# mantasu/face-crop-plus

Measured on AMD Instinct MI355X. Metric: faces/sec end-to-end (detect+align+crop), higher is better.
Workload: dtype f16x3; 1 GPU; RetinaFace detect + 5-pt align/crop, batch=32/GPU synthetic 1024x1024 RGB, strategy=largest, det_threshold=0.6, output 256x256, detector on 2 HIP streams x 16 images; global_batch=32, image_size=1024, parallelism=dp1

## Files before the change

### face-crop-plus_amd/_native.py

```python
from __future__ import annotations

import ctypes as C
import os

_HERE = os.path.dirname(os.path.abspath(__file__))
LIB_PATH = os.path.join(_HERE, "csrc", "libfcp_hip.so")
ABI_VERSION = 15

c_f32p = C.c_void_p
_lib = None


class ConvDesc(C.Structure):
    _fields_ = [
        ("in_", C.c_void_p), ("w", C.c_void_p), ("bias", C.c_void_p), ("out", C.c_void_p),
        ("res1", C.c_void_p), ("res2", C.c_void_p), ("wscale", C.c_void_p), ("in2", C.c_void_p),
        ("n", C.c_int32), ("in_h", C.c_int32), ("in_w", C.c_int32),
        ("cin", C.c_int32), ("in_ld", C.c_int32), ("in_up2", C.c_int32),
        ("cout", C.c_int32), ("kh", C.c_int32), ("kw", C.c_int32),
        ("stride", C.c_int32), ("pad", C.c_int32),
        ("out_h", C.c_int32), ("out_w", C.c_int32), ("out_ld", C.c_int32),
        ("tile_n", C.c_int32), ("cin4", C.c_int32),
        ("act_slope", C.c_float), ("alpha", C.c_float), ("alpha2", C.c_float),
        ("res1_pre", C.c_int32), ("res1_ld", C.c_int32), ("res1_h", C.c_int32),
        ("res1_w", C.c_int32), ("res2_ld", C.c_int32), ("precision", C.c_int32),
        ("in_fmt", C.c_int32), ("out_fmt", C.c_int32), ("res1_fmt", C.c_int32), ("res2_fmt", C.c_int32),
        ("tile_m", C.c_int32), ("cin2", C.c_int32), ("in2_ld", C.c_int32), ("in2_h", C.c_int32),
        ("in2_w", C.c_int32), ("in2_stride", C.c_int32), ("flags", C.c_int32), ("cu_budget", C.c_int32),
        ("band_top", C.c_int32), ("band_bottom", C.c_int32),
    ]


CONV_FLAT_ADDR = 1
CONV_BALANCE_TAIL = 2
CHAIN_OUT_EVEN_ONLY = 1


class ChainDesc(C.Structure):
    _fields_ = [(k, C.c_void_p) for k in ("t1", "w2", "ws2", "b2", "w3", "ws3", "b3", "res", "out", "w1n", "ws1n",
                                          "b1n", "t1n", "t1b")] + \
               [(k, C.c_int32) for k in ("n", "h", "w", "c", "cn", "t1_ld", "res_ld", "out_ld", "t1n_ld", "nout", "tile_m", "flags",
                                         "cb", "t1b_ld", "t1b_h", "t1b_w", "t1b_stride")]


_P, _I, _F, _L = C.c_void_p, C.c_int, C.c_float, C.c_int64
SIGNATURES = {
    "fcp_conv2d_nhwc_f32": [C.POINTER(ConvDesc), _P],
    "fcp_bottleneck_chain_f16x3": [C.POINTER(ChainDesc), _P],
    "fcp_u8_to_nhwc4_f32": [_P, _P, _L, C.POINTER(C.c_float), _F, _P],
# ... 83 lines not shown
```

### face-crop-plus_amd/csrc/fcp_conv.hip

```cpp
#include "fcp_conv_common.h"

#include <cstdlib>

using namespace fcp_conv;

namespace {

constexpr int LDK = 32;


typedef unsigned int u32x4 __attribute__((ext_vector_type(4)));

__device__ __forceinline__ f32x4 buf_load16(__amdgpu_buffer_rsrc_t rsrc, unsigned voff) {
  return __builtin_bit_cast(f32x4, __builtin_amdgcn_raw_buffer_load_b128(rsrc, (int)voff, 0, 0));
}

template <int BN, bool CIN4, bool BUF>
__global__ void __launch_bounds__(256, (BN == 128 ? 2 : (BN == 64 ? 3 : 4))) conv_igemm_f32(const ConvK p) {
  constexpr int WAVES_N = (BN == 32) ? 1 : 2;
  constexpr int WAVES_M = 4 / WAVES_N;
  constexpr int WTM = BM / WAVES_M;
  constexpr int WTN = BN / WAVES_N;
  constexpr int TM = WTM / 32, TN = WTN / 32;
  constexpr int A_LD = BM / 32;
// ... 211 lines not shown
                (!d->res1 || (d->res1_h == d->out_h && d->res1_w == d->out_w)) || halo_wide,
                "conv: the halo-tile kernel needs a 3x3 / stride 1 / pad 1 conv with cin >= 64, cout <= 64 (cout %% 8 == 0) on the "
                "fp16x3 path with a split32 input, no second source, no resized residual");
  if (halo_wide)
    FCP_REQUIRE(d->precision == 1 && d->in_fmt == 1 && !d->cin4 && d->kh == 3 && d->kw == 3 && d->stride == 1 &&
                d->pad == 1 && d->cout % 8 == 0 && d->cin >= 64 && d->cin % 64 == 0 && !d->in2 &&
                ((d->tile_n == 64 && d->cout <= 64 && (!d->res1 || (d->res1_h == d->out_h && d->res1_w == d->out_w))) ||
                 (d->tile_n == 128 && d->cout <= 128 && !d->res1 && !d->res2)),
                "conv: the wide halo-tile kernel (tile_m 1, tile_n 64 / 128) needs a 3x3 / stride 1 / pad 1 conv with cin %% 64 == 0, "
                "cout <= tile_n (cout %% 8 == 0; no residuals above 64 filters) on the fp16x3 path with a split32 input");
  FCP_REQUIRE(d->tile_n == 32 || d->tile_n == 64 || d->tile_n == 128 || (big && (d->tile_n == 256 || d->tile_n == 192)),
              "conv: tile_n must be 32/64/128 (or 192 / 256 with tile_m 256)");
  if (big)
    FCP_REQUIRE(d->precision == 1 && d->in_fmt == 1 && !d->cin4 && !d->in_up2 && d->cout % 8 == 0 && d->tile_n >= 128,
                "conv: 256-row tiles need the fp16x3 path on a split32 input (no cin4 / in_up2), cout %% 8 == 0, tile_n 128/256");
  FCP_REQUIRE(d->kh >= 1 && d->kw >= 1 && d->stride >= 1 && d->pad >= 0, "conv: bad filter geometry");
  FCP_REQUIRE(d->kh * d->kw <= 32 || d->cin4, "conv: at most 32 filter taps (kh*kw) outside cin4 mode");
  FCP_REQUIRE(d->in_ld % 4 == 0 && ((uintptr_t)d->in & 15) == 0, "conv: input must be 16-byte aligned, in_ld %% 4 == 0");
  FCP_REQUIRE(((uintptr_t)d->w & 15) == 0, "conv: filter must be 16-byte aligned");
  if (d->cin4) {
    FCP_REQUIRE(d->cin <= 4 && d->in_ld == 4 && d->kw <= 8, "conv: cin4 mode needs cin<=4, in_ld==4, kw<=8");
  } else {
    FCP_REQUIRE(d->cin % 32 == 0 && d->cin > 0, "conv: cin must be a multiple of 32 (got %d)", d->cin);
  }
  FCP_REQUIRE(d->band_top >= 0 && d->band_bottom >= 0 && d->band_top <= d->pad && d->band_bottom <= d->pad &&
              ((d->band_top | d->band_bottom) == 0 || (d->stride == 1 && !d->in2)),
              "conv: band_top / band_bottom must lie in 0..pad (stride-1 convs without a second source only)");
  const int eh = (d->in_h - d->band_top - d->band_bottom + 2 * d->pad - d->kh) / d->stride + 1;
  const int ew = (d->in_w + 2 * d->pad - d->kw) / d->stride + 1;
  FCP_REQUIRE(eh == d->out_h && ew == d->out_w, "conv: output size %dx%d does not match geometry %dx%d",
// ... 39 lines not shown
    FCP_REQUIRE(d->res1_h > 0 && d->res1_w > 0 && d->res1_ld > 0, "conv: res1 geometry missing");
    if (d->res1_h != d->out_h || d->res1_w != d->out_w) {
      k.res1_resize = 1;
      k.res1_sh = (float)d->res1_h / (float)d->out_h;
      k.res1_sw = (float)d->res1_w / (float)d->out_w;
    }
  }
  if (d->res2) FCP_REQUIRE(d->res2_ld > 0, "conv: res2_ld missing");
  k.vec_ok = (d->out_ld % 4 == 0) && (((uintptr_t)d->out & 15) == 0);
  if (d->res1) k.vec_ok = k.vec_ok && (d->res1_ld % 4 == 0) && (((uintptr_t)d->res1 & 15) == 0);
  if (d->res2) k.vec_ok = k.vec_ok && (d->res2_ld % 4 == 0) && (((uintptr_t)d->res2 & 15) == 0);
  static const int nt_env = getenv("FCP_NT_STORE") ? atoi(getenv("FCP_NT_STORE")) : 1;
  k.nt_store = nt_env;
  k.balance = (d->flags & FCP_CONV_BALANCE_TAIL) ? 1 : 0;
  k.cu_budget = d->cu_budget;
  k.mfull = 0; k.tail_rows = 0; k.round_size = 0;
  k.in2 = nullptr; k.in2_bytes = 0; k.csplit = d->cin; k.in2_ld = 0; k.ph2 = 0; k.pw2 = 0; k.stride2 = 1;
  if (d->in2) {
    FCP_REQUIRE(d->precision == 1 && d->in_fmt == 1 && !d->cin4 && !d->in_up2 && d->kh == 1 && d->kw == 1 && d->pad == 0,
                "conv: a second source needs a 1x1 / pad 0 conv on the fp16x3 path with split32 inputs");
    FCP_REQUIRE(d->cin2 > 0 && d->cin2 < d->cin && d->cin2 % 32 == 0 && d->in2_ld % 32 == 0 && d->in2_ld >= d->cin2 &&
                ((uintptr_t)d->in2 & 127) == 0, "conv: in2 must be a 32-channel-group aligned split32 view, 0 < cin2 < cin");
    FCP_REQUIRE(d->in2_stride >= 1 && d->in2_h > 0 && d->in2_w > 0 && (long)(d->out_h - 1) * d->in2_stride < d->in2_h &&
                (long)(d->out_w - 1) * d->in2_stride < d->in2_w, "conv: in2 geometry does not cover the output grid");
    const unsigned long in2_bytes = (unsigned long)d->n * d->in2_h * d->in2_w * d->in2_ld * 4ul;
    FCP_REQUIRE(in2_bytes < 0xFFFFFFF0ul, "conv: in2 must be below 4 GiB");
    k.in2 = d->in2; k.in2_bytes = (unsigned)in2_bytes; k.csplit = d->cin - d->cin2; k.in2_ld = d->in2_ld;
    k.ph2 = d->in2_h; k.pw2 = d->in2_w; k.stride2 = d->in2_stride;
  }
  k.grid_m = fcp_cdiv(M, BM);
  k.grid_n = fcp_cdiv(d->cout, d->tile_n);
// ... 8 lines not shown
    FCP_REQUIRE(d->wscale != nullptr, "conv: precision 1 needs wscale");
    k.in_bytes = (unsigned)in_bytes;
    k.w_bytes = (unsigned)w_bytes;
    if (halo) {
      k.grid_n = 1;
      const unsigned long out_bytes = (unsigned long)M * d->out_ld * 4ul;
      FCP_REQUIRE(out_bytes < 0xFFFFFFF0ul, "conv(halo): the output view must span less than 4 GiB");
      FCP_REQUIRE(d->wscale != nullptr && ((uintptr_t)d->wscale & 15) == 0 && ((uintptr_t)d->bias & 15) == 0,
                  "conv(halo): wscale / bias must be 16-byte aligned");
      k.in2_bytes = (unsigned)out_bytes;
      k.w_bytes = (unsigned)((unsigned long)fcp_cdiv(d->cout, 128) * 128ul * k.wrow * 4ul);
      return halo_wide ? launch_f16x3_halo_wide(k, s) : launch_f16x3_halo(k, s);
    }
    if (big) {
      k.w_bytes = (unsigned)((unsigned long)fcp_cdiv(d->cout, 128) * 128ul * k.wrow * 4ul);
      return launch_f16x3_big(k, d->tile_n, s);
    }
    if (k.in_fmt == 1 && !d->cin4) return launch_f16x3_dma(k, d->tile_n, s);
    return launch_f16x3(k, d->tile_n, d->cin4 != 0, s);
  }
  k.in_bytes = buf ? (unsigned)in_bytes : 0u;
  k.w_bytes = buf ? (unsigned)w_bytes : 0u;
#define FCP_DISPATCH(BN_)                                                             \
  do {                                                                                \
    if (d->cin4) return buf ? launch<BN_, true, true>(k, s) : launch<BN_, true, false>(k, s); \
    return buf ? launch<BN_, false, true>(k, s) : launch<BN_, false, false>(k, s);   \
  } while (0)
  switch (d->tile_n) {
    case 32: FCP_DISPATCH(32);
    case 64: FCP_DISPATCH(64);
// ... 5 lines not shown
```

### face-crop-plus_amd/csrc/fcp_conv_common.h

```cpp
#pragma once
#include <type_traits>
#include "fcp_common.h"
#include "fcp_hip.h"

typedef float f32x16 __attribute__((ext_vector_type(16)));
typedef float f32x4 __attribute__((ext_vector_type(4)));


constexpr int FCP_AUX_A = 0;
constexpr int FCP_AUX_B = 0;

namespace fcp_conv {

constexpr int BM = 128;
constexpr int BK = 32;

struct ConvK {
  const float* in;
  const float* w;
  const float* bias;
  float* out;
  const float* res1;
  const float* res2;
  int n, in_h, in_w, ph, pw, cin, in_ld, in_up2;
// ... 3 lines not shown
  float act_slope, alpha, alpha2;
  int res1_pre, res1_ld, res1_h, res1_w, res1_resize, res2_ld;
  float res1_sh, res1_sw;
  int grid_m, grid_n, vec_ok;
  unsigned in_bytes, w_bytes;
  const float* wscale;
  int in_fmt, out_fmt, res1_fmt, res2_fmt;
  const float* in2;
  unsigned in2_bytes;
  int csplit, in2_ld, ph2, pw2, stride2;
  int nt_store;
  int balance, cu_budget;
  int mfull, tail_rows, round_size;
  int big_tiles;
  int big_persist;
};


struct TapPiece {
  unsigned base, mask;
};

template <bool CIN4>
__device__ __forceinline__ TapPiece make_tap_piece(const ConvK& p, unsigned pbase, int hi0, int wi0, unsigned chan_off) {
  TapPiece t;
  t.base = ((pbase + (unsigned)(hi0 * p.pw + wi0)) * (unsigned)p.in_ld + chan_off) * 4u;
  t.mask = 0u;
  const int taps = CIN4 ? p.kh : p.kh * p.kw;
  for (int q = 0; q < taps; ++q) {
    const int kh_i = CIN4 ? q : q / p.kw;
// ... 202 lines not shown
        r.a[g] = *reinterpret_cast<const u32x4_t*>(p.res1 + m * p.res1_ld + co);
        r.b[g] = *reinterpret_cast<const u32x4_t*>(p.res1 + m * p.res1_ld + co + 4);
      }
    }
  }
}

template <int I, int N, typename F>
__device__ __forceinline__ void fcp_static_for(F&& f) {
  if constexpr (I < N) {
    f(std::integral_constant<int, I>{});
    fcp_static_for<I + 1, N>(f);
  }
}

template <int TM, int TN, int WTM, int WTN>
__device__ __forceinline__ void conv_epilogue_regs(const ConvK& p, f32x16 (&acc)[TM][TN], int m_start, int m_end, int tm_act, int co_tile,
                                                   int co_end, int wm, int wn, int lane, int hw) {
    const int lp = lane & 15, lg = lane >> 4;
  auto swap32 = [](float& x, float& y) {
    const auto r = __builtin_amdgcn_permlane32_swap(__float_as_uint(x), __float_as_uint(y), false, false);
    const unsigned r0 = r[0], r1 = r[1];
    x = __uint_as_float(r0); y = __uint_as_float(r1);
  };
  auto swap16 = [](float& x, float& y) {
    const auto r = __builtin_amdgcn_permlane16_swap(__float_as_uint(x), __float_as_uint(y), false, false);
    const unsigned r0 = r[0], r1 = r[1];
    x = __uint_as_float(r0); y = __uint_as_float(r1);
  };
  constexpr int GI = TM < 2 ? TM : 2;
  constexpr int NGI = (TM + GI - 1) / GI;
  constexpr int NG = TN * NGI;
  u32x4_t pend_a[GI][2], pend_b[GI][2];
  auto row_of = [&](int i, int set) { return m_start + wm * WTM + i * 32 + 16 * set + lp; };
  auto chan_of = [&](int jj) { return co_tile + wn * WTN + jj * 32 + 8 * lg; };
  auto flush = [&](auto gc) {
    constexpr int g = decltype(gc)::value, jj = g / NGI, i0 = (g % NGI) * GI;
    const int co = chan_of(jj);
    fcp_static_for<0, GI>([&](auto ic) {
      constexpr int i = i0 + decltype(ic)::value;
      if constexpr (i < TM) {
        fcp_static_for<0, 2>([&](auto sc) {
          constexpr int set = decltype(sc)::value;
          const int mi = row_of(i, set);
          if (i < tm_act && mi < m_end && co < co_end) {
            if (p.out_fmt == 1) {
              char* ob = reinterpret_cast<char*>(p.out) + (long)mi * p.out_ld * 4 + split_chan_off(co);
              *reinterpret_cast<u32x4_t*>(ob) = pend_a[i - i0][set];
              *reinterpret_cast<u32x4_t*>(ob + 64) = pend_b[i - i0][set];
            } else {
              float* dst = p.out + (long)mi * p.out_ld + co;
              *reinterpret_cast<u32x4_t*>(dst) = pend_a[i - i0][set];
              *reinterpret_cast<u32x4_t*>(dst + 4) = pend_b[i - i0][set];
            }
          }
        });
      }
    });
  };
  fcp_static_for<0, NG>([&](auto gc) {
    constexpr int g = decltype(gc)::value, j = g / NGI, i0 = (g % NGI) * GI;
    const int co = chan_of(j);
    const bool cok = co < co_end;
    const int cc = cok ? co : co_tile;
    u32x4_t r1a[GI][2], r1b[GI][2];
    if (p.res1 != nullptr) {
      fcp_static_for<0, GI>([&](auto ic) {
        constexpr int i = i0 + decltype(ic)::value;
        if constexpr (i < TM) {
          fcp_static_for<0, 2>([&](auto sc) {
            constexpr int set = decltype(sc)::value;
            const int mi = row_of(i, set);
            const long m = (i < tm_act && mi < m_end && cok) ? (long)mi : (long)m_start;
            long rpix = m;
            if (p.res1_resize) {
              const int ni = (int)(m / hw);
              const int rem = (int)(m - (long)ni * hw);
              const int ho = rem / p.out_w;
              const int wo = rem - ho * p.out_w;
              int sh = (int)floorf(ho * p.res1_sh);
              int sw = (int)floorf(wo * p.res1_sw);
              sh = sh < p.res1_h - 1 ? sh : p.res1_h - 1;
              sw = sw < p.res1_w - 1 ? sw : p.res1_w - 1;
              rpix = ((long)ni * p.res1_h + sh) * p.res1_w + sw;
            }
            if (p.res1_fmt == 1) {
              const char* pb = reinterpret_cast<const char*>(p.res1) + rpix * p.res1_ld * 4 + split_chan_off(cc);
              r1a[i - i0][set] = *reinterpret_cast<const u32x4_t*>(pb);
// ... 32 lines not shown
        });
        fcp_static_for<0, 2>([&](auto sc) {
          constexpr int set = decltype(sc)::value;
          float (&v)[8] = set == 0 ? va : vb;
          float r1[8], r2[8];
          if (p.res1 != nullptr) {
            if (p.res1_fmt == 1) {
              join8(r1a[i - i0][set], r1b[i - i0][set], r1);
            } else {
              const f32x4 fa = __builtin_bit_cast(f32x4, r1a[i - i0][set]), fb = __builtin_bit_cast(f32x4, r1b[i - i0][set]);
              r1[0] = fa[0]; r1[1] = fa[1]; r1[2] = fa[2]; r1[3] = fa[3]; r1[4] = fb[0]; r1[5] = fb[1]; r1[6] = fb[2]; r1[7] = fb[3];
            }
          }
          if (p.res2 != nullptr) {
            const int mi = row_of(i, set);
            load8(p.res2, (i < tm_act && mi < m_end && cok) ? (long)mi : (long)m_start, p.res2_ld, cc, p.res2_fmt, r2);
          }
#pragma unroll
          for (int e = 0; e < 8; ++e) {
            float x = v[e] * ws8[e] + bias8[e];
            if (p.res1 != nullptr && p.res1_pre) x += r1[e];
            x = x >= 0.f ? x : x * p.act_slope;
            x = x * p.alpha;
            if (p.res1 != nullptr && !p.res1_pre) x += r1[e];
            if (p.res2 != nullptr) x = x * p.alpha2 + r2[e];
            v[e] = x;
          }
          if (p.out_fmt == 1) {
            split8(f32x4{v[0], v[1], v[2], v[3]}, f32x4{v[4], v[5], v[6], v[7]}, pend_a[i - i0][set], pend_b[i - i0][set]);
          } else {
            pend_a[i - i0][set] = __builtin_bit_cast(u32x4_t, f32x4{v[0], v[1], v[2], v[3]});
// ... 113 lines not shown
```

### face-crop-plus_amd/csrc/fcp_conv_f16x3_big.hip

```cpp
#include "fcp_conv_common.h"

#include <type_traits>

using namespace fcp_conv;

namespace {

typedef _Float16 f16x8 __attribute__((ext_vector_type(8)));

constexpr int BMB = 256;
constexpr int NT = 512;
constexpr int ROWB = 128;
constexpr int STAGE = 1 << 16;

template <int IMM>
__device__ __forceinline__ f16x8 lds_read128(unsigned addr) {
  f16x8 v;
  asm volatile("ds_read_b128 %0, %1 offset:%2" : "=v"(v) : "v"(addr), "n"(IMM));
  return v;
}

template <int I, int N, typename F>
__device__ __forceinline__ void static_for(F&& f) {
  if constexpr (I < N) {
    f(std::integral_constant<int, I>{});
    static_for<I + 1, N>(f);
  }
}

template <int BN>
__global__ void __launch_bounds__(NT, 1) conv_igemm_f16x3_big(const ConvK p) {
  constexpr int WAVES_N = BN == 256 ? 4 : 2;
  constexpr int WAVES_M = 8 / WAVES_N;
  constexpr int WTM = BMB / WAVES_M, WTN = BN / WAVES_N;
  constexpr int TM = WTM / 32, TN = WTN / 32;
  constexpr int A_LD = BMB / 64, B_LD = BN / 64;

  extern __shared__ __attribute__((aligned(16))) float smem[];
  char* lds = reinterpret_cast<char*>(smem);

  const int nb = p.big_tiles;
  int vb = blockIdx.x;
  int tile_n = 0, m_start = 0, m_end = 0;
  auto decode = [&](int bid) {
    const int rbase = (bid / p.round_size) * p.round_size;
    const int nr = nb - rbase < p.round_size ? nb - rbase : p.round_size;
    const int bi = bid - rbase;
    const int q8 = nr >> 3, r8 = nr & 7, xcd = bi & 7;
    const int logical = rbase + (xcd < r8 ? xcd * (q8 + 1) : r8 * (q8 + 1) + (xcd - r8) * q8) + (bi >> 3);
    tile_n = logical % p.grid_n;
    const int tile_m = logical / p.grid_n;
// ... 2 lines not shown
    m_end = m_start + m_rows < p.M ? m_start + m_rows : p.M;
  };
  decode(vb);

  const int tid = threadIdx.x;
  const int lane = tid & 63;
  const int wave_u = __builtin_amdgcn_readfirstlane(tid >> 6);
  const int wm = wave_u / WAVES_N, wn = wave_u % WAVES_N;
  const int lrow = tid >> 3;
  const int csrc = (tid & 7) ^ (((lrow >> 1) & 7) ^ ((lrow & 1) << 2));

  const int hw = p.out_h * p.out_w;
  TapPiece tp[A_LD];
  unsigned base2[A_LD];
  unsigned woff[B_LD];
  auto setup_tile = [&]() {
#pragma unroll
  for (int i = 0; i < A_LD; ++i) {
    const int m = m_start + lrow + 64 * i;
    unsigned pbase = 0;
    int hi0 = -(1 << 28), wi0 = 0;
    base2[i] = 0xFFFFFFFFu;
    if (m < m_end) {
      const int ni = m / hw;
      const int rem = m - ni * hw;
      const int ho = rem / p.out_w;
      const int wo = rem - ho * p.out_w;
      pbase = (unsigned)(ni * p.ph * p.pw);
      hi0 = ho * p.stride - p.pad_h;
      wi0 = wo * p.stride - p.pad;
      if (p.in2 != nullptr)
        base2[i] = (((unsigned)(ni * p.ph2 + ho * p.stride2) * (unsigned)p.pw2 + (unsigned)(wo * p.stride2)) * (unsigned)p.in2_ld +
                    (unsigned)(csrc * 4)) * 4u;
    }
    tp[i] = make_tap_piece<false>(p, pbase, hi0, wi0, (unsigned)(csrc * 4));
  }
#pragma unroll
    for (int i = 0; i < B_LD; ++i) woff[i] = (unsigned)(((tile_n * BN + lrow + 64 * i) * p.wrow + csrc * 4) * 4);
  };
  setup_tile();
  __amdgpu_buffer_rsrc_t rs_in2 = __builtin_amdgcn_make_buffer_rsrc(const_cast<float*>(p.in2 ? p.in2 : p.in), 0, p.in2_bytes, 0x00020000);
  __amdgpu_buffer_rsrc_t rs_in = __builtin_amdgcn_make_buffer_rsrc(const_cast<float*>(p.in), 0, p.in_bytes, 0x00020000);
  __amdgpu_buffer_rsrc_t rs_w = __builtin_amdgcn_make_buffer_rsrc(const_cast<float*>(p.w), 0, p.w_bytes, 0x00020000);
  unsigned rowoff[A_LD];
  auto set_tap = [&](int tap, int kh_i, int kw_i) {
    const unsigned tapoff = (unsigned)((kh_i * p.pw + kw_i) * p.in_ld) * 4u;
#pragma unroll
    for (int i = 0; i < A_LD; ++i) rowoff[i] = ((tp[i].mask >> tap) & 1u) ? tp[i].base + tapoff : 0xFFFFFFFFu;
  };
  int tap = 0, kh_i = 0, kw_i = 0, c0 = 0;
  auto advance = [&]() {
// ... 16 lines not shown
      }
    } else {
#pragma unroll
      for (int i = 0; i < A_LD; ++i) {
        const unsigned ro = rowoff[i];
        __builtin_amdgcn_raw_ptr_buffer_load_lds(rs_in, (__attribute__((address_space(3))) void*)(a + 64 * i * ROWB), 16,
                                                 (int)(ro == 0xFFFFFFFFu ? 0xFFFFFFFFu : ro + (unsigned)(c0 * 4)), 0, 0, FCP_AUX_A);
      }
    }
#pragma unroll
    for (int i = 0; i < B_LD; ++i)
      __builtin_amdgcn_raw_ptr_buffer_load_lds(rs_w, (__attribute__((address_space(3))) void*)(b + 64 * i * ROWB), 16,
                                               (int)(woff[i] + (unsigned)(kt * BK * 4)), 0, 0, FCP_AUX_B);
  };

  f32x16 acc[TM][TN];

  const unsigned lds0 = (unsigned)(size_t)(__attribute__((address_space(3))) char*)lds;
  const int rsw = (((lane & 31) >> 1) & 7) ^ ((lane & 1) << 2);
  const int half = lane >> 5;
  const unsigned arow = lds0 + (unsigned)((wm * WTM + (lane & 31)) * ROWB);
  const unsigned brow = lds0 + (unsigned)((BMB + wn * WTN + (lane & 31)) * ROWB);
  unsigned aH[2], aL[2], bH[2], bL[2];
#pragma unroll
  for (int s = 0; s < 2; ++s) {
    const unsigned oh = (unsigned)(((2 * s + half) ^ rsw) << 4), ol = (unsigned)(((4 + 2 * s + half) ^ rsw) << 4);
    aH[s] = arow + oh; aL[s] = arow + ol;
    bH[s] = brow + oh; bL[s] = brow + ol;
  }

  auto prefetch_tile = [&]() {
    tap = 0; kh_i = 0; kw_i = 0; c0 = 0;
    set_tap(0, 0, 0);
    dma_slice(0, 0);
    if (p.ktiles > 1) {
      advance();
      dma_slice(1, 1);
    }
  };
  prefetch_tile();
  int tm_act = 0;
  auto main_loop = [&](auto tma_c) {
    constexpr int TMA = decltype(tma_c)::value;
    f16x8 fah[2][TMA > 0 ? TMA : 1], fal[2][TMA > 0 ? TMA : 1], fbh[2][TN], fbl[2][TN];
  auto read_frags = [&](auto set_c, unsigned stage_xor) {
    constexpr int set = decltype(set_c)::value;
    static_for<0, TMA>([&](auto ic) {
      constexpr int i = decltype(ic)::value;
      fah[set][i] = lds_read128<i * 32 * ROWB>(aH[set] ^ stage_xor);
      fal[set][i] = lds_read128<i * 32 * ROWB>(aL[set] ^ stage_xor);
    });
    static_for<0, TN>([&](auto jc) {
      constexpr int j = decltype(jc)::value;
      fbh[set][j] = lds_read128<j * 32 * ROWB>(bH[set] ^ stage_xor);
      fbl[set][j] = lds_read128<j * 32 * ROWB>(bL[set] ^ stage_xor);
    });
  };
  constexpr std::integral_constant<int, 0> SET0{};
  constexpr std::integral_constant<int, 1> SET1{};
  auto mfmas_reads = [&](auto cs_c, auto ls_c, unsigned stage_xor) {
    constexpr int cs = decltype(cs_c)::value, ls = decltype(ls_c)::value;
    constexpr int NM = 3 * TMA * TN, NR = 2 * TMA + 2 * TN;
    static_for<0, NM>([&](auto mc) {
      constexpr int m = decltype(mc)::value;
      constexpr int g = m / (TMA * TN), i = (m % (TMA * TN)) / TN, j = m % TN;
      if constexpr (g == 0) acc[i][j] = __builtin_amdgcn_mfma_f32_32x32x16_f16(fbh[cs][j], fal[cs][i], acc[i][j], 0, 0, 0);
      else if constexpr (g == 1) acc[i][j] = __builtin_amdgcn_mfma_f32_32x32x16_f16(fbl[cs][j], fah[cs][i], acc[i][j], 0, 0, 0);
      else acc[i][j] = __builtin_amdgcn_mfma_f32_32x32x16_f16(fbh[cs][j], fah[cs][i], acc[i][j], 0, 0, 0);
      __builtin_amdgcn_sched_barrier(0);
      static_for<0, NR>([&](auto rc) {
        constexpr int r = decltype(rc)::value;
        if constexpr (((r + 1) * NM) / NR - 1 == m
        ) {
          if constexpr (r < 2 * TMA) {
            constexpr int ii = r / 2;
            if constexpr (r % 2 == 0) fah[ls][ii] = lds_read128<ii * 32 * ROWB>(aH[ls] ^ stage_xor);
            else fal[ls][ii] = lds_read128<ii * 32 * ROWB>(aL[ls] ^ stage_xor);
          } else {
            constexpr int jj = (r - 2 * TMA) / 2;
            if constexpr (r % 2 == 0) fbh[ls][jj] = lds_read128<jj * 32 * ROWB>(bH[ls] ^ stage_xor);
            else fbl[ls][jj] = lds_read128<jj * 32 * ROWB>(bL[ls] ^ stage_xor);
          }
          __builtin_amdgcn_sched_barrier(0);
        }
      });
    });
  };

  read_frags(SET0, 0u);
  asm volatile("s_waitcnt lgkmcnt(0)" ::: "memory");
  __builtin_amdgcn_sched_barrier(0);

  unsigned sx = 0u;
  for (int kt = 0; kt < p.ktiles; ++kt) {
    mfmas_reads(SET0, SET1, sx);
    __builtin_amdgcn_sched_barrier(0);
    asm volatile("s_waitcnt lgkmcnt(0)" ::: "memory");
    asm volatile("s_waitcnt vmcnt(0)" ::: "memory");
    __builtin_amdgcn_s_barrier();
    __builtin_amdgcn_sched_barrier(0);
    const bool dma_first = wave_u >= 4;
    if (dma_first && kt + 2 < p.ktiles) {
      advance();
      dma_slice(kt + 2, kt & 1);
    }
    __builtin_amdgcn_sched_barrier(0);
    mfmas_reads(SET1, SET0, sx ^ (unsigned)STAGE);
    __builtin_amdgcn_sched_barrier(0);
    if (!dma_first && kt + 2 < p.ktiles) {
      advance();
      dma_slice(kt + 2, kt & 1);
    }
    __builtin_amdgcn_sched_barrier(0);
    asm volatile("s_waitcnt lgkmcnt(0)" ::: "memory");
    __builtin_amdgcn_sched_barrier(0);
    sx ^= (unsigned)STAGE;
  }
  };
  for (;;) {
  asm volatile("s_waitcnt vmcnt(0)" ::: "memory");
  __builtin_amdgcn_s_barrier();
  __builtin_amdgcn_sched_barrier(0);
  tm_act = (m_end - m_start - wm * WTM + 31) >> 5;
  tm_act = __builtin_amdgcn_readfirstlane(tm_act < 0 ? 0 : (tm_act > TM ? TM : tm_act));
#pragma unroll
  for (int i = 0; i < TM; ++i)
#pragma unroll
    for (int j = 0; j < TN; ++j)
#pragma unroll
      for (int e = 0; e < 16; ++e) acc[i][j][e] = 0.f;
  static_for<0, TM + 1>([&](auto tc) {
    if (tm_act == decltype(tc)::value) main_loop(tc);
  });
  asm volatile("s_waitcnt vmcnt(0)" ::: "memory");
  __builtin_amdgcn_s_barrier();

  const int e_tile_n = tile_n, e_m_start = m_start, e_m_end = m_end, e_tm_act = tm_act;
  const bool more = p.big_persist && vb + p.round_size < nb;
  if (more) {
    vb += p.round_size;
    decode(vb);
    setup_tile();
    prefetch_tile();
  }
  conv_epilogue_regs<TM, TN, WTM, WTN>(p, acc, e_m_start, e_m_end, e_tm_act, e_tile_n * BN,
                                       (e_tile_n + 1) * BN < p.cout ? (e_tile_n + 1) * BN : p.cout, wm, wn, lane, hw);
  if (!more) break;
  }
}

template <int BN>
int launch(ConvK k, hipStream_t s) {
  const size_t lds = 2 * (size_t)STAGE;
  FCP_LDS_OPT_IN((&conv_igemm_f16x3_big<BN>), lds);
  k.grid_n = fcp_cdiv(k.cout, BN);
  int cus = k.cu_budget > 0 ? k.cu_budget : fcp_cu_count();
  cus = cus < 8 ? 8 : (cus & ~7);
  k.round_size = cus;
  const int mt = fcp_cdiv(k.M, BMB);
  k.mfull = mt;
  k.tail_rows = BMB;
  k.grid_m = mt;
  if (k.balance) {
    const long tiles = (long)mt * k.grid_n;
    const long full_rounds = tiles / cus;
    const int mfull = (int)((full_rounds * cus) / k.grid_n);
    const long rem = (long)k.M - (long)mfull * BMB;
    if (rem > 0) {
      const long slots = cus / k.grid_n > 0 ? cus / k.grid_n : 1;
      long r = ((rem + slots - 1) / slots + 31) / 32 * 32;
      r = r < 32 ? 32 : r;
      if (r < BMB) {
        k.mfull = mfull;
        k.tail_rows = (int)r;
        k.grid_m = mfull + (int)((rem + r - 1) / r);
      }
    }
  }
  k.big_tiles = k.grid_m * k.grid_n;
  static const int persist_env = getenv("FCP_BIG_PERSIST") ? atoi(getenv("FCP_BIG_PERSIST")) : -1;
  k.big_persist = persist_env < 0 ? (k.cu_budget == 0) : (persist_env != 0);
  hipLaunchKernelGGL((conv_igemm_f16x3_big<BN>), dim3(k.big_persist && k.big_tiles > k.round_size ? k.round_size : k.big_tiles), dim3(NT), lds, s, k);
  FCP_LAUNCH_OK();
  return 0;
}

}

namespace fcp_conv {

int launch_f16x3_big(const ConvK& k, int tile_n, hipStream_t s) {
  return tile_n == 256 ? launch<256>(k, s) : tile_n == 192 ? launch<192>(k, s) : launch<128>(k, s);
}

}
```

### face-crop-plus_amd/engine.py

```python
from __future__ import annotations

import contextlib
import ctypes as C
import os
import threading
from dataclasses import dataclass

import numpy as np
import torch

from . import _native as N
from . import torch_ops as T

BN_EPS = 1e-5
COUT_PAD = 128


class Act:
    __slots__ = ("buf", "c0", "c", "fmt")

    def __init__(self, buf: torch.Tensor, c0: int = 0, c: int | None = None, fmt: int = 0):
        assert buf.dim() == 4 and buf.dtype == torch.float32 and buf.is_contiguous()
        self.buf, self.c0, self.fmt = buf, c0, fmt
        self.c = buf.shape[3] - c0 if c is None else c
# ... 564 lines not shown
    d.flags = flags
    d.cu_budget = cu_budget
    d.band_top, d.band_bottom = band
    if res1 is not None:
        d.res1_ld, d.res1_h, d.res1_w = res1.ld, res1.h, res1.w
    if res2 is not None:
        d.res2_ld = res2.ld
    return d


def conv(pc: PackedConv, x: Act, out: Act | None = None, *, act_slope: float = 1.0,
         alpha: float = 1.0, res1: Act | None = None, res1_pre: bool = True,
         res2: Act | None = None, alpha2: float = 1.0, in_up2: bool = False,
         tile_n: int | None = None, out_fmt: int = 0, tile_m: int | None = None,
         x2: Act | None = None, x2_stride: int = 1, flat: bool = False, balance_tail: bool = False,
         band: tuple[int, int] = (0, 0)) -> Act:
    assert x.c + (x2.c if x2 is not None else 0) == pc.cin, f"conv expects {pc.cin} input channels, got {x.c}"
    in_h, in_w = (x.h * 2, x.w * 2) if in_up2 else (x.h, x.w)
    oh = (in_h - band[0] - band[1] + 2 * pc.pad - pc.kh) // pc.stride + 1
    ow = (in_w + 2 * pc.pad - pc.kw) // pc.stride + 1
    if out is None:
        out = Act.empty(x.n, oh, ow, pc.cout, x.buf.device, out_fmt)
    assert (out.n, out.h, out.w, out.c) == (x.n, oh, ow, pc.cout), "conv: bad output view"
    if (x.fmt or out.fmt or (res1 is not None and res1.fmt) or (res2 is not None and res2.fmt)) and pc.precision != 1:
        raise ValueError("split32 tensors can only be used with filters packed for the fp16x3 path")
    assert x2 is None or (x2.fmt == 1 and x.fmt == 1 and x2.n == x.n), "two-source convs take split32 tensors"
    assert res1 is None or (res1.c == pc.cout and res1.n == x.n)
    assert res2 is None or (res2.n, res2.h, res2.w, res2.c) == (x.n, oh, ow, pc.cout)
    m = x.n * oh * ow
    tm, tn = tile_m or 128, tile_n or _pick_tile_n(pc.cout, m)
    flags = (N.CONV_FLAT_ADDR if flat else 0) | (N.CONV_BALANCE_TAIL if balance_tail else 0)
    cu = getattr(_budget, "cus", 0)
    desc = lambda o: _conv_desc(pc, x, o, x2, x2_stride, res1, res1_pre, res2, alpha, alpha2, act_slope, in_up2, band,
                                tm, tn, flags, cu)
    big_ok = (pc.precision == 1 and x.fmt == 1 and not pc.cin4 and not in_up2 and pc.cout % 8 == 0
              and pc.cout >= 128 and m >= 256 * 64)
    halo_ok = (pc.precision == 1 and x.fmt == 1 and not pc.cin4 and (pc.kh, pc.kw, pc.stride, pc.pad) == (3, 3, 1, 1)
               and pc.cout <= 64 and pc.cout % 8 == 0 and pc.cin >= 64 and x2 is None and (res1 is None or (res1.h, res1.w) == (oh, ow)))
    wide_ok = (pc.precision == 1 and x.fmt == 1 and not pc.cin4 and (pc.kh, pc.kw, pc.stride, pc.pad) == (3, 3, 1, 1)
               and pc.cout % 8 == 0 and pc.cin % 64 == 0 and x2 is None and 64 < pc.cout <= 128 and res1 is None and res2 is None)
    if tile_n is None and tile_m is None and (pc.cout > 64 or halo_ok):
        key = (pc.cin, pc.cout, pc.kh, pc.kw, pc.stride, m, int(in_up2), res1 is not None, res2 is not None,
               pc.precision, x.fmt, out.fmt, None if x2 is None else (x2.c, x2_stride), cu)
        best = Autotune.choose(key, tile_candidates(pc.cout, halo_ok, wide_ok, big_ok),
                               lambda: desc(_alias_safe_out(out, x, x2, res1, res2)))
        if best is not None:
# ... 280 lines not shown
```

### include/fcp_hip.h

```cpp
#ifndef FCP_HIP_H
#define FCP_HIP_H

#include <stdint.h>

#ifdef __cplusplus
extern "C" {
#endif

#define FCP_ABI_VERSION 15

typedef void* fcp_stream_t;

int fcp_abi_version(void);
const char* fcp_last_error(void);

typedef struct fcp_conv_desc {
  const float* in;
  const void* w;
  const float* bias;
  float* out;
  const float* res1;
  const float* res2;
  const float* wscale;
  const float* in2;
// ... 5 lines not shown
  int32_t tile_n;
  int32_t cin4;
  float act_slope, alpha, alpha2;
  int32_t res1_pre, res1_ld, res1_h, res1_w, res2_ld;
  int32_t precision;
  int32_t in_fmt, out_fmt, res1_fmt, res2_fmt;
  int32_t tile_m;
  int32_t cin2, in2_ld, in2_h, in2_w, in2_stride;
  int32_t flags;
  int32_t cu_budget;
  int32_t band_top, band_bottom;
} fcp_conv_desc;

#define FCP_CONV_FLAT_ADDR 1
#define FCP_CONV_BALANCE_TAIL 2

int fcp_conv2d_nhwc_f32(const fcp_conv_desc* desc, fcp_stream_t stream);

typedef struct fcp_chain_desc {
  const float* t1;
  const void* w2;  const float* ws2;  const float* b2;
  const void* w3;  const float* ws3;  const float* b3;
  const float* res;
  float* out;
  const void* w1n; const float* ws1n; const float* b1n;
  float* t1n;
  const float* t1b;
  int32_t n, h, w, c, cn;
  int32_t t1_ld, res_ld, out_ld, t1n_ld;
  int32_t nout;
// ... 171 lines not shown
```

Measured before the change: 1454 faces/s.

## Add halo-operand form to 256-row fp16x3 implicit-GEMM conv for 3x3 stride-1

Adds a halo variant of the big 256-row conv kernel. Instead of re-fetching the input once per 3x3 tap, it loads an 8x32 output patch plus a one-pixel halo (10x34 rows) into LDS once per channel slice and reads all nine taps from it with swizzled offsets. The epilogue remaps patch rows to output pixels. The halo form is the default whenever the shape qualifies, unless FCP_BIG_HALO=0 or the per_tap flag is set. This cuts global/L2 input traffic for 3x3 convs, in exchange for more complex LDS addressing, a different LDS footprint and coarser tail tiles.

```diff
diff --git a/face-crop-plus_amd/_native.py b/face-crop-plus_amd/_native.py
--- a/face-crop-plus_amd/_native.py
+++ b/face-crop-plus_amd/_native.py
@@ -33,6 +33,8 @@
 
 CONV_FLAT_ADDR = 1
 CONV_BALANCE_TAIL = 2
+CONV_BIG_HALO = 4
+CONV_BIG_PER_TAP = 8
 CHAIN_OUT_EVEN_ONLY = 1
 
 
diff --git a/face-crop-plus_amd/csrc/fcp_conv.hip b/face-crop-plus_amd/csrc/fcp_conv.hip
--- a/face-crop-plus_amd/csrc/fcp_conv.hip
+++ b/face-crop-plus_amd/csrc/fcp_conv.hip
@@ -249,6 +249,14 @@
   if (big)
     FCP_REQUIRE(d->precision == 1 && d->in_fmt == 1 && !d->cin4 && !d->in_up2 && d->cout % 8 == 0 && d->tile_n >= 128,
                 "conv: 256-row tiles need the fp16x3 path on a split32 input (no cin4 / in_up2), cout %% 8 == 0, tile_n 128/256");
+  const bool halo_form_ok = big && d->kh == 3 && d->kw == 3 && d->stride == 1 && d->pad == 1 && d->out_h % 8 == 0 &&
+                            d->out_w % 32 == 0 && !d->in2 && !d->in_up2 && d->band_top == 0 && d->band_bottom == 0;
+  FCP_REQUIRE(!(d->flags & FCP_CONV_BIG_HALO) || !(d->flags & FCP_CONV_BIG_PER_TAP),
+              "conv: FCP_CONV_BIG_HALO and FCP_CONV_BIG_PER_TAP exclude each other");
+  FCP_REQUIRE(!(d->flags & FCP_CONV_BIG_PER_TAP) || big, "conv: FCP_CONV_BIG_PER_TAP is an option of the 256-row kernel (tile_m 256)");
+  FCP_REQUIRE(!(d->flags & FCP_CONV_BIG_HALO) || halo_form_ok,
+              "conv: FCP_CONV_BIG_HALO needs tile_m 256 and a 3x3 / stride 1 / pad 1 conv with out_h %% 8 == 0, out_w %% 32 == 0, "
+              "no second source, no in_up2, no row band");
   FCP_REQUIRE(d->kh >= 1 && d->kw >= 1 && d->stride >= 1 && d->pad >= 0, "conv: bad filter geometry");
   FCP_REQUIRE(d->kh * d->kw <= 32 || d->cin4, "conv: at most 32 filter taps (kh*kw) outside cin4 mode");
   FCP_REQUIRE(d->in_ld % 4 == 0 && ((uintptr_t)d->in & 15) == 0, "conv: input must be 16-byte aligned, in_ld %% 4 == 0");
@@ -318,7 +326,7 @@
   k.nt_store = nt_env;
   k.balance = (d->flags & FCP_CONV_BALANCE_TAIL) ? 1 : 0;
   k.cu_budget = d->cu_budget;
-  k.mfull = 0; k.tail_rows = 0; k.round_size = 0;
+  k.mfull = 0; k.tail_rows = 0; k.round_size = 0; k.big_form = -1;
   k.in2 = nullptr; k.in2_bytes = 0; k.csplit = d->cin; k.in2_ld = 0; k.ph2 = 0; k.pw2 = 0; k.stride2 = 1;
   if (d->in2) {
     FCP_REQUIRE(d->precision == 1 && d->in_fmt == 1 && !d->cin4 && !d->in_up2 && d->kh == 1 && d->kw == 1 && d->pad == 0,
@@ -357,6 +365,7 @@
     }
     if (big) {
       k.w_bytes = (unsigned)((unsigned long)fcp_cdiv(d->cout, 128) * 128ul * k.wrow * 4ul);
+      k.big_form = !halo_form_ok ? -1 : (d->flags & FCP_CONV_BIG_HALO) ? 1 : (d->flags & FCP_CONV_BIG_PER_TAP) ? 2 : 0;
       return launch_f16x3_big(k, d->tile_n, s);
     }
     if (k.in_fmt == 1 && !d->cin4) return launch_f16x3_dma(k, d->tile_n, s);
diff --git a/face-crop-plus_amd/csrc/fcp_conv_common.h b/face-crop-plus_amd/csrc/fcp_conv_common.h
--- a/face-crop-plus_amd/csrc/fcp_conv_common.h
+++ b/face-crop-plus_amd/csrc/fcp_conv_common.h
@@ -41,6 +41,7 @@
   int mfull, tail_rows, round_size;
   int big_tiles;
   int big_persist;
+  int big_form;
 };
 
 
@@ -273,10 +274,18 @@
   }
 }
 
-template <int TM, int TN, int WTM, int WTN>
+template <int TM, int TN, int WTM, int WTN, bool PATCH = false>
 __device__ __forceinline__ void conv_epilogue_regs(const ConvK& p, f32x16 (&acc)[TM][TN], int m_start, int m_end, int tm_act, int co_tile,
-                                                   int co_end, int wm, int wn, int lane, int hw) {
+                                                   int co_end, int wm, int wn, int lane, int hw, int patch_pix = 0) {
     const int lp = lane & 15, lg = lane >> 4;
+  auto pix_of = [&](int mi) -> long {
+    if constexpr (PATCH) {
+      const int r = mi - m_start;
+      return (long)(patch_pix + (r >> 5) * p.out_w + (r & 31));
+    } else {
+      return (long)mi;
+    }
+  };
   auto swap32 = [](float& x, float& y) {
     const auto r = __builtin_amdgcn_permlane32_swap(__float_as_uint(x), __float_as_uint(y), false, false);
     const unsigned r0 = r[0], r1 = r[1];
@@ -304,11 +313,11 @@
           const int mi = row_of(i, set);
           if (i < tm_act && mi < m_end && co < co_end) {
             if (p.out_fmt == 1) {
-              char* ob = reinterpret_cast<char*>(p.out) + (long)mi * p.out_ld * 4 + split_chan_off(co);
+              char* ob = reinterpret_cast<char*>(p.out) + pix_of(mi) * p.out_ld * 4 + split_chan_off(co);
               *reinterpret_cast<u32x4_t*>(ob) = pend_a[i - i0][set];
               *reinterpret_cast<u32x4_t*>(ob + 64) = pend_b[i - i0][set];
             } else {
-              float* dst = p.out + (long)mi * p.out_ld + co;
+              float* dst = p.out + pix_of(mi) * p.out_ld + co;
               *reinterpret_cast<u32x4_t*>(dst) = pend_a[i - i0][set];
               *reinterpret_cast<u32x4_t*>(dst + 4) = pend_b[i - i0][set];
             }
@@ -330,7 +339,7 @@
           fcp_static_for<0, 2>([&](auto sc) {
             constexpr int set = decltype(sc)::value;
             const int mi = row_of(i, set);
-            const long m = (i < tm_act && mi < m_end && cok) ? (long)mi : (long)m_start;
+            const long m = pix_of((i < tm_act && mi < m_end && cok) ? mi : m_start);
             long rpix = m;
             if (p.res1_resize) {
               const int ni = (int)(m / hw);
@@ -393,7 +402,7 @@
           }
           if (p.res2 != nullptr) {
             const int mi = row_of(i, set);
-            load8(p.res2, (i < tm_act && mi < m_end && cok) ? (long)mi : (long)m_start, p.res2_ld, cc, p.res2_fmt, r2);
+            load8(p.res2, pix_of((i < tm_act && mi < m_end && cok) ? mi : m_start), p.res2_ld, cc, p.res2_fmt, r2);
           }
 #pragma unroll
           for (int e = 0; e < 8; ++e) {
diff --git a/face-crop-plus_amd/csrc/fcp_conv_f16x3_big.hip b/face-crop-plus_amd/csrc/fcp_conv_f16x3_big.hip
--- a/face-crop-plus_amd/csrc/fcp_conv_f16x3_big.hip
+++ b/face-crop-plus_amd/csrc/fcp_conv_f16x3_big.hip
@@ -12,6 +12,13 @@
 constexpr int NT = 512;
 constexpr int ROWB = 128;
 constexpr int STAGE = 1 << 16;
+constexpr int HALO_W = 34;
+constexpr int HALO_ROWS = 10 * HALO_W;
+constexpr int HALO_A = HALO_ROWS * ROWB;
+constexpr int HALO_PIECES = (HALO_ROWS + 7) / 8;
+constexpr int HALO_Q = (HALO_PIECES + 7) / 8;
+constexpr int HALO_B_OFF = 2 * HALO_A;
+__device__ __forceinline__ int swz(int row) { return ((row >> 1) & 7) ^ ((row & 1) << 2); }
 
 template <int IMM>
 __device__ __forceinline__ f16x8 lds_read128(unsigned addr) {
@@ -20,6 +27,18 @@
   return v;
 }
 
+template <int X, int IMM>
+__device__ __forceinline__ f16x8 lds_read128_ax(unsigned addr, unsigned soff) {
+  f16x8 v;
+  unsigned t;
+  if constexpr (X != 0)
+    asm volatile("v_add_u32 %1, %3, %2\n\tv_xor_b32 %1, %4, %1\n\tds_read_b128 %0, %1 offset:%5"
+                 : "=v"(v), "=&v"(t) : "v"(addr), "s"(soff), "n"(X), "n"(IMM));
+  else
+    asm volatile("v_add_u32 %1, %3, %2\n\tds_read_b128 %0, %1 offset:%4" : "=v"(v), "=&v"(t) : "v"(addr), "s"(soff), "n"(IMM));
+  return v;
+}
+
 template <int I, int N, typename F>
 __device__ __forceinline__ void static_for(F&& f) {
   if constexpr (I < N) {
@@ -28,13 +47,15 @@
   }
 }
 
-template <int BN>
+template <int BN, bool HALO>
 __global__ void __launch_bounds__(NT, 1) conv_igemm_f16x3_big(const ConvK p) {
   constexpr int WAVES_N = BN == 256 ? 4 : 2;
   constexpr int WAVES_M = 8 / WAVES_N;
   constexpr int WTM = BMB / WAVES_M, WTN = BN / WAVES_N;
   constexpr int TM = WTM / 32, TN = WTN / 32;
   constexpr int A_LD = BMB / 64, B_LD = BN / 64;
+  constexpr unsigned BSTG = BN * ROWB;
+  static_assert(!HALO || HALO_B_OFF + 2 * BN * ROWB <= 160 * 1024, "halo-operand form: LDS budget");
 
   extern __shared__ __attribute__((aligned(16))) float smem[];
   char* lds = reinterpret_cast<char*>(smem);
@@ -67,7 +88,28 @@
   TapPiece tp[A_LD];
   unsigned base2[A_LD];
   unsigned woff[B_LD];
+  unsigned abase[HALO_Q];
+  int patch_pix = 0;
   auto setup_tile = [&]() {
+  if constexpr (HALO) {
+    const int patch = m_start >> 8, py0 = (m_start & 255) >> 5, nrows = (m_end - m_start) >> 5;
+    const int pcols = p.out_w >> 5, ppi = (p.out_h >> 3) * pcols;
+    const int ni = patch / ppi, prem = patch - ni * ppi;
+    const int pr = prem / pcols, pc = prem - pr * pcols;
+    const int y0 = pr * 8 + py0, x0 = pc * 32;
+    patch_pix = (ni * p.out_h + y0) * p.out_w + x0;
+#pragma unroll
+    for (int q = 0; q < HALO_Q; ++q) {
+      const int j = wave_u + 8 * q;
+      const int r0 = 8 * j < HALO_ROWS - 8 ? 8 * j : HALO_ROWS - 8;
+      const int hr = r0 + (lane >> 3);
+      const int hy = hr / HALO_W, hx = hr - hy * HALO_W;
+      const int y = y0 - 1 + hy, x = x0 - 1 + hx;
+      const bool ok = hy < nrows + 2 && (unsigned)y < (unsigned)p.in_h && (unsigned)x < (unsigned)p.in_w;
+      const int cs = (lane & 7) ^ swz(hx);
+      abase[q] = ok ? ((unsigned)((ni * p.ph + y) * p.pw + x) * (unsigned)p.in_ld + (unsigned)(cs * 4)) * 4u : 0xFFFFFFFFu;
+    }
+  } else {
 #pragma unroll
   for (int i = 0; i < A_LD; ++i) {
     const int m = m_start + lrow + 64 * i;
@@ -88,6 +130,7 @@
     }
     tp[i] = make_tap_piece<false>(p, pbase, hi0, wi0, (unsigned)(csrc * 4));
   }
+  }
 #pragma unroll
     for (int i = 0; i < B_LD; ++i) woff[i] = (unsigned)(((tile_n * BN + lrow + 64 * i) * p.wrow + csrc * 4) * 4);
   };
@@ -134,13 +177,31 @@
                                                (int)(woff[i] + (unsigned)(kt * BK * 4)), 0, 0, FCP_AUX_B);
   };
 
+  auto dma_b = [&](int kt, unsigned bst) {
+    char* b = lds + HALO_B_OFF + bst + wave_u * 8 * ROWB;
+#pragma unroll
+    for (int i = 0; i < B_LD; ++i)
+      __builtin_amdgcn_raw_ptr_buffer_load_lds(rs_w, (__attribute__((address_space(3))) void*)(b + 64 * i * ROWB), 16,
+                                               (int)(woff[i] + (unsigned)(kt * BK * 4)), 0, 0, FCP_AUX_B);
+  };
+  auto dma_a = [&](auto q_c, int cs, unsigned ast) {
+    constexpr int q = decltype(q_c)::value;
+    const int j = wave_u + 8 * q;
+    if (j < HALO_PIECES) {
+      const int r0 = 8 * j < HALO_ROWS - 8 ? 8 * j : HALO_ROWS - 8;
+      const unsigned ro = abase[q];
+      __builtin_amdgcn_raw_ptr_buffer_load_lds(rs_in, (__attribute__((address_space(3))) void*)(lds + ast + r0 * ROWB), 16,
+                                               (int)(ro == 0xFFFFFFFFu ? 0xFFFFFFFFu : ro + (unsigned)(cs * 128)), 0, 0, FCP_AUX_A);
+    }
+  };
+
   f32x16 acc[TM][TN];
 
   const unsigned lds0 = (unsigned)(size_t)(__attribute__((address_space(3))) char*)lds;
   const int rsw = (((lane & 31) >> 1) & 7) ^ ((lane & 1) << 2);
   const int half = lane >> 5;
   const unsigned arow = lds0 + (unsigned)((wm * WTM + (lane & 31)) * ROWB);
-  const unsigned brow = lds0 + (unsigned)((BMB + wn * WTN + (lane & 31)) * ROWB);
+  const unsigned brow = lds0 + (HALO ? (unsigned)(HALO_B_OFF + (wn * WTN + (lane & 31)) * ROWB) : (unsigned)((BMB + wn * WTN + (lane & 31)) * ROWB));
   unsigned aH[2], aL[2], bH[2], bL[2];
 #pragma unroll
   for (int s = 0; s < 2; ++s) {
@@ -148,14 +209,28 @@
     aH[s] = arow + oh; aL[s] = arow + ol;
     bH[s] = brow + oh; bL[s] = brow + ol;
   }
+  unsigned aaddr[3];
+  if constexpr (HALO) {
+#pragma unroll
+    for (int kw = 0; kw < 3; ++kw) {
+      const int hx = (lane & 31) + kw;
+      aaddr[kw] = lds0 + (unsigned)((wm * TM * HALO_W + hx) * ROWB + ((half ^ swz(hx)) << 4));
+    }
+  }
 
   auto prefetch_tile = [&]() {
-    tap = 0; kh_i = 0; kw_i = 0; c0 = 0;
-    set_tap(0, 0, 0);
-    dma_slice(0, 0);
-    if (p.ktiles > 1) {
-      advance();
-      dma_slice(1, 1);
+    if constexpr (HALO) {
+      static_for<0, HALO_Q>([&](auto qc) { dma_a(qc, 0, 0u); });
+      dma_b(0, 0u);
+      dma_b(1, BSTG);
+    } else {
+      tap = 0; kh_i = 0; kw_i = 0; c0 = 0;
+      set_tap(0, 0, 0);
+      dma_slice(0, 0);
+      if (p.ktiles > 1) {
+        advance();
+        dma_slice(1, 1);
+      }
     }
   };
   prefetch_tile();
@@ -178,7 +253,32 @@
   };
   constexpr std::integral_constant<int, 0> SET0{};
   constexpr std::integral_constant<int, 1> SET1{};
-  auto mfmas_reads = [&](auto cs_c, auto ls_c, unsigned stage_xor) {
+  auto rd_tap = [&](auto ls_c, auto rc, unsigned stage_xor) {
+    constexpr int ls = decltype(ls_c)::value, r = decltype(rc)::value;
+    if constexpr (r < 2 * TMA) {
+      constexpr int ii = r / 2;
+      if constexpr (r % 2 == 0) fah[ls][ii] = lds_read128<ii * 32 * ROWB>(aH[ls] ^ stage_xor);
+      else fal[ls][ii] = lds_read128<ii * 32 * ROWB>(aL[ls] ^ stage_xor);
+    } else {
+      constexpr int jj = (r - 2 * TMA) / 2;
+      if constexpr (r % 2 == 0) fbh[ls][jj] = lds_read128<jj * 32 * ROWB>(bH[ls] ^ stage_xor);
+      else fbl[ls][jj] = lds_read128<jj * 32 * ROWB>(bL[ls] ^ stage_xor);
+    }
+  };
+  auto rd_halo = [&](auto ls_c, auto rc, auto tap_c, unsigned aoff, unsigned boff) {
+    constexpr int ls = decltype(ls_c)::value, r = decltype(rc)::value, tp_ = decltype(tap_c)::value;
+    constexpr int kh = tp_ / 3, kw = tp_ % 3;
+    if constexpr (r < 2 * TMA) {
+      constexpr int ii = r / 2;
+      if constexpr (r % 2 == 0) fah[ls][ii] = lds_read128_ax<(ls ? 0x20 : 0), (ii + kh) * HALO_W * ROWB>(aaddr[kw], aoff);
+      else fal[ls][ii] = lds_read128_ax<(ls ? 0x60 : 0x40), (ii + kh) * HALO_W * ROWB>(aaddr[kw], aoff);
+    } else {
+      constexpr int jj = (r - 2 * TMA) / 2;
+      if constexpr (r % 2 == 0) fbh[ls][jj] = lds_read128<jj * 32 * ROWB>(bH[ls] + boff);
+      else fbl[ls][jj] = lds_read128<jj * 32 * ROWB>(bL[ls] + boff);
+    }
+  };
+  auto mfmas_reads = [&](auto cs_c, auto ls_c, auto&& rd) {
     constexpr int cs = decltype(cs_c)::value, ls = decltype(ls_c)::value;
     constexpr int NM = 3 * TMA * TN, NR = 2 * TMA + 2 * TN;
     static_for<0, NM>([&](auto mc) {
@@ -192,28 +292,62 @@
         constexpr int r = decltype(rc)::value;
         if constexpr (((r + 1) * NM) / NR - 1 == m
         ) {
-          if constexpr (r < 2 * TMA) {
-            constexpr int ii = r / 2;
-            if constexpr (r % 2 == 0) fah[ls][ii] = lds_read128<ii * 32 * ROWB>(aH[ls] ^ stage_xor);
-            else fal[ls][ii] = lds_read128<ii * 32 * ROWB>(aL[ls] ^ stage_xor);
-          } else {
-            constexpr int jj = (r - 2 * TMA) / 2;
-            if constexpr (r % 2 == 0) fbh[ls][jj] = lds_read128<jj * 32 * ROWB>(bH[ls] ^ stage_xor);
-            else fbl[ls][jj] = lds_read128<jj * 32 * ROWB>(bL[ls] ^ stage_xor);
-          }
+          rd(rc);
           __builtin_amdgcn_sched_barrier(0);
         }
       });
     });
   };
 
+  if constexpr (HALO) {
+    constexpr int NR = 2 * TMA + 2 * TN;
+    constexpr std::integral_constant<int, 0> TAP0{};
+    static_for<0, NR>([&](auto rc) { rd_halo(SET0, rc, TAP0, 0u, 0u); });
+    asm volatile("s_waitcnt lgkmcnt(0)" ::: "memory");
+    __builtin_amdgcn_sched_barrier(0);
+    const bool dma_first = wave_u >= 4;
+    unsigned aoff = 0u, bcur = 0u;
+    int kt = 0;
+    for (int c = 0; c < p.ctiles; ++c) {
+      const unsigned aoff_n = (unsigned)HALO_A - aoff;
+      const bool next_slice = c + 1 < p.ctiles;
+      static_for<0, 9>([&](auto tc) {
+        constexpr int t = decltype(tc)::value;
+        constexpr std::integral_constant<int, (t + 1) % 9> tnext{};
+        const unsigned bnext = BSTG - bcur;
+        mfmas_reads(SET0, SET1, [&](auto rc) { rd_halo(SET1, rc, tc, aoff, bcur); });
+        __builtin_amdgcn_sched_barrier(0);
+        asm volatile("s_waitcnt lgkmcnt(0)" ::: "memory");
+        asm volatile("s_waitcnt vmcnt(0)" ::: "memory");
+        __builtin_amdgcn_s_barrier();
+        __builtin_amdgcn_sched_barrier(0);
+        auto dma = [&]() {
+          if (kt + 2 < p.ktiles) dma_b(kt + 2, bcur);
+          if constexpr (t < HALO_Q) {
+            if (next_slice) dma_a(tc, c + 1, aoff_n);
+          }
+        };
+        if (dma_first) dma();
+        __builtin_amdgcn_sched_barrier(0);
+        mfmas_reads(SET1, SET0, [&](auto rc) { rd_halo(SET0, rc, tnext, t == 8 ? aoff_n : aoff, bnext); });
+        __builtin_amdgcn_sched_barrier(0);
+        if (!dma_first) dma();
+        __builtin_amdgcn_sched_barrier(0);
+        asm volatile("s_waitcnt lgkmcnt(0)" ::: "memory");
+        __builtin_amdgcn_sched_barrier(0);
+        bcur = bnext;
+        ++kt;
+      });
+      aoff = aoff_n;
+    }
+  } else {
   read_frags(SET0, 0u);
   asm volatile("s_waitcnt lgkmcnt(0)" ::: "memory");
   __builtin_amdgcn_sched_barrier(0);
 
   unsigned sx = 0u;
   for (int kt = 0; kt < p.ktiles; ++kt) {
-    mfmas_reads(SET0, SET1, sx);
+    mfmas_reads(SET0, SET1, [&](auto rc) { rd_tap(SET1, rc, sx); });
     __builtin_amdgcn_sched_barrier(0);
     asm volatile("s_waitcnt lgkmcnt(0)" ::: "memory");
     asm volatile("s_waitcnt vmcnt(0)" ::: "memory");
@@ -225,7 +359,7 @@
       dma_slice(kt + 2, kt & 1);
     }
     __builtin_amdgcn_sched_barrier(0);
-    mfmas_reads(SET1, SET0, sx ^ (unsigned)STAGE);
+    mfmas_reads(SET1, SET0, [&](auto rc) { rd_tap(SET0, rc, sx ^ (unsigned)STAGE); });
     __builtin_amdgcn_sched_barrier(0);
     if (!dma_first && kt + 2 < p.ktiles) {
       advance();
@@ -235,6 +369,7 @@
     asm volatile("s_waitcnt lgkmcnt(0)" ::: "memory");
     __builtin_amdgcn_sched_barrier(0);
     sx ^= (unsigned)STAGE;
+  }
   }
   };
   for (;;) {
@@ -255,7 +390,7 @@
   asm volatile("s_waitcnt vmcnt(0)" ::: "memory");
   __builtin_amdgcn_s_barrier();
 
-  const int e_tile_n = tile_n, e_m_start = m_start, e_m_end = m_end, e_tm_act = tm_act;
+  const int e_tile_n = tile_n, e_m_start = m_start, e_m_end = m_end, e_tm_act = tm_act, e_patch_pix = patch_pix;
   const bool more = p.big_persist && vb + p.round_size < nb;
   if (more) {
     vb += p.round_size;
@@ -263,16 +398,16 @@
     setup_tile();
     prefetch_tile();
   }
-  conv_epilogue_regs<TM, TN, WTM, WTN>(p, acc, e_m_start, e_m_end, e_tm_act, e_tile_n * BN,
-                                       (e_tile_n + 1) * BN < p.cout ? (e_tile_n + 1) * BN : p.cout, wm, wn, lane, hw);
+  conv_epilogue_regs<TM, TN, WTM, WTN, HALO>(p, acc, e_m_start, e_m_end, e_tm_act, e_tile_n * BN,
+                                             (e_tile_n + 1) * BN < p.cout ? (e_tile_n + 1) * BN : p.cout, wm, wn, lane, hw, e_patch_pix);
   if (!more) break;
   }
 }
 
-template <int BN>
+template <int BN, bool HALO>
 int launch(ConvK k, hipStream_t s) {
-  const size_t lds = 2 * (size_t)STAGE;
-  FCP_LDS_OPT_IN((&conv_igemm_f16x3_big<BN>), lds);
+  const size_t lds = HALO ? (size_t)(HALO_B_OFF + 2 * BN * ROWB) : 2 * (size_t)STAGE;
+  FCP_LDS_OPT_IN((&conv_igemm_f16x3_big<BN, HALO>), lds);
   k.grid_n = fcp_cdiv(k.cout, BN);
   int cus = k.cu_budget > 0 ? k.cu_budget : fcp_cu_count();
   cus = cus < 8 ? 8 : (cus & ~7);
@@ -290,6 +425,7 @@
       const long slots = cus / k.grid_n > 0 ? cus / k.grid_n : 1;
       long r = ((rem + slots - 1) / slots + 31) / 32 * 32;
       r = r < 32 ? 32 : r;
+      if (HALO) r = r <= 32 ? 32 : r <= 64 ? 64 : r <= 128 ? 128 : BMB;
       if (r < BMB) {
         k.mfull = mfull;
         k.tail_rows = (int)r;
@@ -300,7 +436,7 @@
   k.big_tiles = k.grid_m * k.grid_n;
   static const int persist_env = getenv("FCP_BIG_PERSIST") ? atoi(getenv("FCP_BIG_PERSIST")) : -1;
   k.big_persist = persist_env < 0 ? (k.cu_budget == 0) : (persist_env != 0);
-  hipLaunchKernelGGL((conv_igemm_f16x3_big<BN>), dim3(k.big_persist && k.big_tiles > k.round_size ? k.round_size : k.big_tiles), dim3(NT), lds, s, k);
+  hipLaunchKernelGGL((conv_igemm_f16x3_big<BN, HALO>), dim3(k.big_persist && k.big_tiles > k.round_size ? k.round_size : k.big_tiles), dim3(NT), lds, s, k);
   FCP_LAUNCH_OK();
   return 0;
 }
@@ -310,7 +446,10 @@
 namespace fcp_conv {
 
 int launch_f16x3_big(const ConvK& k, int tile_n, hipStream_t s) {
-  return tile_n == 256 ? launch<256>(k, s) : tile_n == 192 ? launch<192>(k, s) : launch<128>(k, s);
-}
-
-}
+  static const int halo_env = getenv("FCP_BIG_HALO") ? atoi(getenv("FCP_BIG_HALO")) : -1;
+  const bool halo = k.big_form == 1 || (k.big_form == 0 && halo_env != 0);
+  if (halo) return tile_n == 256 ? launch<256, true>(k, s) : tile_n == 192 ? launch<192, true>(k, s) : launch<128, true>(k, s);
+  return tile_n == 256 ? launch<256, false>(k, s) : tile_n == 192 ? launch<192, false>(k, s) : launch<128, false>(k, s);
+}
+
+}
diff --git a/face-crop-plus_amd/engine.py b/face-crop-plus_amd/engine.py
--- a/face-crop-plus_amd/engine.py
+++ b/face-crop-plus_amd/engine.py
@@ -602,7 +602,7 @@
          res2: Act | None = None, alpha2: float = 1.0, in_up2: bool = False,
          tile_n: int | None = None, out_fmt: int = 0, tile_m: int | None = None,
          x2: Act | None = None, x2_stride: int = 1, flat: bool = False, balance_tail: bool = False,
-         band: tuple[int, int] = (0, 0)) -> Act:
+         band: tuple[int, int] = (0, 0), big_form: str | None = None) -> Act:
     assert x.c + (x2.c if x2 is not None else 0) == pc.cin, f"conv expects {pc.cin} input channels, got {x.c}"
     in_h, in_w = (x.h * 2, x.w * 2) if in_up2 else (x.h, x.w)
     oh = (in_h - band[0] - band[1] + 2 * pc.pad - pc.kh) // pc.stride + 1
@@ -618,6 +618,7 @@
     m = x.n * oh * ow
     tm, tn = tile_m or 128, tile_n or _pick_tile_n(pc.cout, m)
     flags = (N.CONV_FLAT_ADDR if flat else 0) | (N.CONV_BALANCE_TAIL if balance_tail else 0)
+    flags |= {None: 0, "halo": N.CONV_BIG_HALO, "per_tap": N.CONV_BIG_PER_TAP}[big_form]
     cu = getattr(_budget, "cus", 0)
     desc = lambda o: _conv_desc(pc, x, o, x2, x2_stride, res1, res1_pre, res2, alpha, alpha2, act_slope, in_up2, band,
                                 tm, tn, flags, cu)
diff --git a/include/fcp_hip.h b/include/fcp_hip.h
--- a/include/fcp_hip.h
+++ b/include/fcp_hip.h
@@ -43,6 +43,8 @@
 
 #define FCP_CONV_FLAT_ADDR 1
 #define FCP_CONV_BALANCE_TAIL 2
+#define FCP_CONV_BIG_HALO 4
+#define FCP_CONV_BIG_PER_TAP 8
 
 int fcp_conv2d_nhwc_f32(const fcp_conv_desc* desc, fcp_stream_t stream);
 
```

After: 1467 faces/s, median of 6. No clear change (+0.9%).
